# Kyaw-Thiha/animal-vision

Hardware: NVIDIA B200
Metric: Mpix/s (higher is better)
Workload: dtype f32

## Files before the change

animal_vision_b200/csrc/k3_uv.cu:

```cuda
#include <algorithm>

#include "avb_common.cuh"

namespace avb {

constexpr int UV_BINS = 2048;
constexpr int UV_NH = 3;
constexpr int UV_NR = 4;
constexpr int UV_MAX_BANDS = 160;
constexpr int UV_THREADS = 256, UV_WARPS = UV_THREADS / 32;
#ifndef UV_RH_ROWS
#define UV_RH_ROWS 64
#endif
constexpr int UV_RH = UV_RH_ROWS;
#ifndef UV_MINB
#define UV_MINB 4
#endif
#ifndef UV_HIST_WAVES
#define UV_HIST_WAVES 1
#endif
constexpr unsigned FULL = 0xffffffffu;

enum { MAP_OPPONENT = 0, MAP_FALSECOLOR = 1, MAP_MATRIX = 2, MAP_PURPLE = 3, MAP_MIXED = 4 };
enum { QS_OPP = 0, QS_UBG = 1, QS_U = 2 };

struct UvFrameStats {
    uint32_t max_bits[3];
    uint32_t pad0;
    double sum[3];
    float rcp[3];
    float pad2[6];
    float scale[3];
    float inv_w[UV_NH];
    uint32_t bin_lo[UV_NR], bin_hi[UV_NR], rank_lo[UV_NR], rank_hi[UV_NR], cand_count[UV_NR];
    float pct[UV_NR];
    uint32_t pad1;
};
static_assert(sizeof(UvFrameStats) % 8 == 0, "stats block must stay 8-byte aligned");

struct UvParams {
    FrameIO io;
    const float *lut;
    float M3[9];
    const float *bands;
    int n_bands;
    float denom_eps;
    int adapt;
    float eps;
    float t0, t1, t2;
    UvFrameStats *stats;
    uint32_t *hist;
    float *planes;
    float *cand;
    long long cap;
    const uint32_t *enc;
    int n_req;
    int req_hist[UV_NR];
    long long k_lo[UV_NR], k_hi[UV_NR];
    float gamma[UV_NR];
    int mapper;
    float map_m[9];
    float anchors[6];
    float mix_alpha;
    float *dbg_catches;
    int aligned_in, aligned_out;
    int no_plane_map;
    int strips_x, strips_y;
};

__device__ __forceinline__ float div_by(float x, float s, float r) {
    const float q = __fmul_rn(x, r);
    return fmaf(fmaf(-q, s, x), r, q);
}

__device__ __noinline__ void band_sum(const float4 *bands, int n_bands, float denom_eps, float c0, float c1, float c2,
                                      float &u, float &b, float &g) {
    float au = 0.f, ab = 0.f, ag = 0.f;
    for (int l = 0; l < n_bands; ++l) {
        const float4 lo = __ldg(bands + 2 * l), hi = __ldg(bands + 2 * l + 1);
        float spec = __fadd_rn(__fadd_rn(__fmul_rn(lo.z, c2), __fmul_rn(lo.y, c1)), __fmul_rn(lo.x, c0));
        spec = fmaxf(__fdiv_rn(spec, denom_eps), 0.f);
        const float rad = __fmul_rn(spec, lo.w);
        au = fmaf(rad, hi.x, au);
        ab = fmaf(rad, hi.y, ab);
        ag = fmaf(rad, hi.z, ag);
    }
    u = au; b = ab; g = ag;
}

template <bool BANDS>
struct Catcher {
    const float *lut_s;
    float m[9];
    const float4 *bands;
    int n_bands;
    float denom_eps;
    float sc[3], rc[3];
    bool divide;

    __device__ __forceinline__ void init_raw(const UvParams &p, const float *lut) {
        lut_s = lut;
#pragma unroll
        for (int i = 0; i < 9; ++i) m[i] = p.M3[i];
        bands = reinterpret_cast<const float4 *>(p.bands);
        n_bands = p.n_bands;
        denom_eps = p.denom_eps;
        sc[0] = sc[1] = sc[2] = 1.f;
        rc[0] = rc[1] = rc[2] = 1.f;
        divide = false;
    }
    __device__ __forceinline__ void init_adapted(const UvParams &p, const UvFrameStats &st, const float *lut) {
        init_raw(p, lut);
#pragma unroll
        for (int k = 0; k < 3; ++k) { sc[k] = st.scale[k]; rc[k] = st.rcp[k]; }
        divide = p.adapt != 0;
    }
    __device__ __forceinline__ void operator()(uint32_t b0, uint32_t b1, uint32_t b2, float &u, float &b, float &g) const {
        from_linear(lut_s[b0], lut_s[b1], lut_s[b2], u, b, g);
    }
    __device__ __forceinline__ void from_linear(float c0, float c1, float c2, float &u, float &b, float &g) const {
        if constexpr (!BANDS) {
            u = m[0] * c0 + m[1] * c1 + m[2] * c2;
            b = m[3] * c0 + m[4] * c1 + m[5] * c2;
            g = m[6] * c0 + m[7] * c1 + m[8] * c2;
            if (divide) {
                u = div_by(u, sc[0], rc[0]);
                b = div_by(b, sc[1], rc[1]);
                g = div_by(g, sc[2], rc[2]);
            }
        } else {
            float au, ab, ag;
            band_sum(bands, n_bands, denom_eps, c0, c1, c2, au, ab, ag);
            if (divide) {
                au = __fdiv_rn(au, sc[0]);
                ab = __fdiv_rn(ab, sc[1]);
                ag = __fdiv_rn(ag, sc[2]);
            }
            u = au; b = ab; g = ag;
        }
    }
};

__device__ __forceinline__ uint32_t byte_k(uint32_t w, int k) { return __byte_perm(w, 0, 0x4440 + k); }

template <class Cat>
__device__ __forceinline__ void catches4(const Cat &cat, const uint32_t (&w)[3], float (&c)[4][3]) {
    cat(byte_k(w[0], 0), byte_k(w[0], 1), byte_k(w[0], 2), c[0][0], c[0][1], c[0][2]);
    cat(byte_k(w[0], 3), byte_k(w[1], 0), byte_k(w[1], 1), c[1][0], c[1][1], c[1][2]);
    cat(byte_k(w[1], 2), byte_k(w[1], 3), byte_k(w[2], 0), c[2][0], c[2][1], c[2][2]);
    cat(byte_k(w[2], 1), byte_k(w[2], 2), byte_k(w[2], 3), c[3][0], c[3][1], c[3][2]);
}

template <int R, class Cat, class Op>
__device__ __forceinline__ void uv_walk(const UvParams &p, const Cat &cat, const uint8_t *src, int xs, int ys, int rows, Op &op) {
    constexpr int OFF = R ? 4 : 0;
    const int lane = threadIdx.x & 31;
    const int H = p.io.H, W = p.io.W;
    const int gx = xs - OFF + 4 * lane;
    const bool fast = p.aligned_in && gx >= 0 && gx + 3 < W;
    int xi[4];
#pragma unroll
    for (int j = 0; j < 4; ++j) xi[j] = 3 * reflect101(gx + j, W);
    const bool lane_ok = (R == 0) || (lane >= 1 && lane <= 30);

    auto load = [&](int i, uint32_t(&w)[3]) {
        const uint8_t *row = src + (int64_t)reflect101(ys + i, H) * p.io.in_rs;
        if (fast) {
            const uint32_t *q = reinterpret_cast<const uint32_t *>(row + 3 * gx);
            w[0] = __ldg(q); w[1] = __ldg(q + 1); w[2] = __ldg(q + 2);
        } else {
            uint32_t b[12];
#pragma unroll
            for (int j = 0; j < 4; ++j) {
                const uint8_t *q = row + xi[j];
                b[3 * j] = q[0]; b[3 * j + 1] = q[1]; b[3 * j + 2] = q[2];
            }
#pragma unroll
            for (int k = 0; k < 3; ++k) w[k] = b[4 * k] | (b[4 * k + 1] << 8) | (b[4 * k + 2] << 16) | (b[4 * k + 3] << 24);
        }
    };

    float acc[2 * R + 1][4][3];
#pragma unroll
    for (int m = 0; m < 2 * R + 1; ++m)
#pragma unroll
        for (int j = 0; j < 4; ++j)
#pragma unroll
            for (int k = 0; k < 3; ++k) acc[m][j][k] = 0.f;
    uint32_t w[3], wn[3] = {0u, 0u, 0u};
    const int n_iter = rows + 2 * R;
    const float tp[3] = {p.t0, p.t1, p.t2};
    load(-R, w);
    for (int i = 0; i < n_iter; ++i) {
        if (i + 1 < n_iter) load(i + 1 - R, wn);
        float c[4][3];
        catches4(cat, w, c);
        float v[4][3];
        if constexpr (R == 0) {
#pragma unroll
            for (int j = 0; j < 4; ++j)
#pragma unroll
                for (int k = 0; k < 3; ++k) v[j][k] = c[j][k];
        } else {
#pragma unroll
            for (int k = 0; k < 3; ++k) {
                float e[8];
                e[1] = __shfl_up_sync(FULL, c[3][k], 1);
                e[6] = __shfl_down_sync(FULL, c[0][k], 1);
                if (R == 2) {
                    e[0] = __shfl_up_sync(FULL, c[2][k], 1);
                    e[7] = __shfl_down_sync(FULL, c[1][k], 1);
                } else {
                    e[0] = e[7] = 0.f;
                }
#pragma unroll
                for (int j = 0; j < 4; ++j) e[2 + j] = c[j][k];
#pragma unroll
                for (int j = 0; j < 4; ++j) {
                    float h = fmaf(tp[1], e[1 + j] + e[3 + j], tp[0] * e[2 + j]);
                    if (R == 2) h = fmaf(tp[2], e[j] + e[4 + j], h);
                    v[j][k] = fmaf(tp[R], h, acc[0][j][k]);
#pragma unroll
                    for (int m = 0; m < 2 * R - 1; ++m) {
                        const int d = (R - 1 - m) < 0 ? -(R - 1 - m) : (R - 1 - m);
                        acc[m][j][k] = fmaf(tp[d], h, acc[m + 1][j][k]);
                    }
                    acc[2 * R - 1][j][k] = tp[R] * h;
                }
            }
        }
        if (i >= 2 * R) op(ys + i - 2 * R, gx, v, lane_ok);
#pragma unroll
        for (int k = 0; k < 3; ++k) w[k] = wn[k];
    }
}

template <int R>
__device__ __forceinline__ void strip_of(const UvParams &p, int task, int &xs, int &ys, int &rows) {
    constexpr int SW = R ? 120 : 128;
    const int sy = task / p.strips_x, sx = task - sy * p.strips_x;
    xs = sx * SW;
    ys = sy * UV_RH;
    rows = min(UV_RH, p.io.H - ys);
}

__device__ __forceinline__ float sqrt_sfu(float x) {
#ifdef UV_SQRT_RN
    return __fsqrt_rn(x);
#else
    float r;
    asm("sqrt.approx.ftz.f32 %0, %1;" : "=f"(r) : "f"(x));
    return r;
#endif
}

__device__ __forceinline__ float atan2_fast(float y, float x) {
    const float ax = fabsf(x), ay = fabsf(y);
    const float mx = fmaxf(ax, ay), mn = fminf(ax, ay);
    const float a = mx > 0.f ? __fdividef(mn, mx) : 0.f;
    const float s = a * a;
    float r = 0.0028662257f;
    r = fmaf(r, s, -0.0161657367f);
    r = fmaf(r, s, 0.0429096138f);
    r = fmaf(r, s, -0.0752896400f);
    r = fmaf(r, s, 0.1065626393f);
    r = fmaf(r, s, -0.1420889944f);
    r = fmaf(r, s, 0.1999355085f);
// ... 8 lines not shown
__device__ __forceinline__ float opp_hue(const float (&c)[3]) {
    const float O1 = c[2] - c[1], O2 = c[1] - c[0];
    const float PI_F = 3.14159274101257324f;
    const float ang = PRECISE ? atan2f(O2, O1) : atan2_fast(O2, O1);
    return div_by(__fadd_rn(ang, PI_F), 6.28318548202514648f, 0.159154936671257019f);
}

template <int QS, bool PRECISE = false>
__device__ __forceinline__ void quantities(const float (&c)[3], float (&q)[UV_NH]) {
    if (QS == QS_OPP) {
        const float O1 = c[2] - c[1], O2 = c[1] - c[0];
        const float r2 = __fadd_rn(__fmul_rn(O1, O1), __fmul_rn(O2, O2));
        q[0] = PRECISE ? __fsqrt_rn(r2) : sqrt_sfu(r2);
        q[1] = div_by(__fadd_rn(__fadd_rn(c[0], c[1]), c[2]), 3.0f, 0.333333343267440796f);
        q[2] = 0.f;
    } else {
        q[0] = c[0]; q[1] = c[1]; q[2] = c[2];
    }
}
template <int QS>
struct QCount { static constexpr int value = QS == QS_OPP ? 2 : (QS == QS_UBG ? 3 : 1); };

__device__ __forceinline__ int bin_of(float v, float inv_w) {
    return min(UV_BINS - 1, max(0, __float2int_rd(v * inv_w)));
}

template <bool BANDS>
__global__ void __launch_bounds__(256) uv_stats_kernel(const __grid_constant__ UvParams p) {
    __shared__ float lut_s[256];
    for (int i = threadIdx.x; i < 256; i += blockDim.x) lut_s[i] = __ldg(p.lut + i);
    __syncthreads();
    const int frame = blockIdx.y;
    const uint8_t *src = p.io.in + (int64_t)frame * p.io.in_fs;
    Catcher<BANDS> cat;
    cat.init_raw(p, lut_s);
    float mx[3] = {0.f, 0.f, 0.f};
    double sm[3] = {0.0, 0.0, 0.0};
    const int W = p.io.W, H = p.io.H;
    const int groups = (W + 3) >> 2;
    for (int y = blockIdx.x; y < H; y += gridDim.x) {
        const uint8_t *row = src + (int64_t)y * p.io.in_rs;
        float rs[3] = {0.f, 0.f, 0.f};
        int gi = threadIdx.x;
        if (p.aligned_in) {
            for (; gi + 3 * (int)blockDim.x < groups - 1; gi += 4 * blockDim.x) {
                uint32_t w[4][3];
#pragma unroll
                for (int u = 0; u < 4; ++u) {
                    const uint32_t *q = reinterpret_cast<const uint32_t *>(row + 12 * (gi + u * (int)blockDim.x));
                    w[u][0] = __ldg(q); w[u][1] = __ldg(q + 1); w[u][2] = __ldg(q + 2);
                }
#pragma unroll
                for (int u = 0; u < 4; ++u) {
                    float c[4][3];
                    catches4(cat, w[u], c);
#pragma unroll
                    for (int j = 0; j < 4; ++j) {
#pragma unroll
                        for (int k = 0; k < 3; ++k) {
                            mx[k] = fmaxf(mx[k], c[j][k]);
                            rs[k] += c[j][k];
                        }
                        if (p.dbg_catches) {
                            float *d = p.dbg_catches + (((int64_t)frame * H + y) * W + 4 * (gi + u * (int)blockDim.x) + j) * 3;
                            d[0] = c[j][0]; d[1] = c[j][1]; d[2] = c[j][2];
                        }
                    }
                }
// ... 21 lines not shown
                    d[0] = c[j][0]; d[1] = c[j][1]; d[2] = c[j][2];
                }
            }
        }
#pragma unroll
        for (int k = 0; k < 3; ++k) sm[k] += (double)rs[k];
    }
    __shared__ float red_m[8][3];
    __shared__ double red_s[8][3];
    const int lane = threadIdx.x & 31, wid = threadIdx.x >> 5;
#pragma unroll
    for (int k = 0; k < 3; ++k) {
        float m = mx[k];
        double s = sm[k];
#pragma unroll
        for (int o = 16; o > 0; o >>= 1) {
            m = fmaxf(m, __shfl_xor_sync(FULL, m, o));
            s += __shfl_xor_sync(FULL, s, o);
        }
        if (lane == 0) { red_m[wid][k] = m; red_s[wid][k] = s; }
    }
    __syncthreads();
    if (threadIdx.x < 3) {
        const int k = threadIdx.x;
        float m = 0.f;
        double s = 0.0;
        for (int w = 0; w < (int)(blockDim.x >> 5); ++w) { m = fmaxf(m, red_m[w][k]); s += red_s[w][k]; }
        UvFrameStats &st = p.stats[frame];
        atomicMax(&st.max_bits[k], __float_as_uint(fmaxf(m, 0.f)));
        atomicAdd(&st.sum[k], s);
    }
}

template <int QS>
__global__ void uv_prep_kernel(const __grid_constant__ UvParams p) {
    const int frame = blockIdx.x * blockDim.x + threadIdx.x;
    if (frame >= p.io.n) return;
    UvFrameStats &st = p.stats[frame];
    const double npx = (double)p.io.H * (double)p.io.W;
    float ub[3];
#pragma unroll
    for (int k = 0; k < 3; ++k) {
        const float mx = __uint_as_float(st.max_bits[k]);
        float s = 1.0f;
        if (p.adapt == 1) s = fmaxf(mx, p.eps);
        else if (p.adapt == 2) s = fmaxf((float)(st.sum[k] / npx), p.eps);
        st.scale[k] = s;
        st.rcp[k] = __frcp_rn(s);
        ub[k] = mx / s * 1.001f + 1e-30f;
    }
    float hb[UV_NH];
    if (QS == QS_OPP) {
        const float a = fmaxf(ub[2], ub[1]), b = fmaxf(ub[1], ub[0]);
        hb[0] = sqrtf(a * a + b * b) * 1.001f;
        hb[1] = (ub[0] + ub[1] + ub[2]) * (1.001f / 3.0f);
        hb[2] = 1.f;
    } else {
        hb[0] = ub[0]; hb[1] = ub[1]; hb[2] = ub[2];
    }
#pragma unroll
    for (int h = 0; h < UV_NH; ++h) st.inv_w[h] = (float)UV_BINS / fmaxf(hb[h], 1e-30f);
}

__host__ __device__ __forceinline__ bool map_from_planes(const UvParams &p) {
    return p.n_req > 0 && (p.io.W & 3) == 0 && p.aligned_out != 0 && !p.no_plane_map;
}

template <int QS>
struct HistOp {
    uint32_t *hs;
    float *planes;
    long long npx;
    float inv_w[UV_NH];
    int W;
    bool vec;
    bool hue_plane;
    __device__ __forceinline__ void operator()(int y, int gx, const float (&v)[4][3], bool ok) {
        if (!ok || gx >= W) return;
        constexpr int NPL = QS == QS_OPP ? 3 : QCount<QS>::value;
        float q[4][UV_NH];
        const bool full = gx + 3 < W;
#pragma unroll
        for (int j = 0; j < 4; ++j) {
            quantities<QS>(v[j], q[j]);
            if (QS == QS_OPP && hue_plane) q[j][2] = opp_hue<false>(v[j]);
        }
        if (full) {
#pragma unroll
            for (int j = 0; j < 4; ++j)
#pragma unroll
                for (int h = 0; h < QCount<QS>::value; ++h) atomicAdd(&hs[h * UV_BINS + bin_of(q[j][h], inv_w[h])], 1u);
        } else {
#pragma unroll
            for (int j = 0; j < 4; ++j)
                if (gx + j < W) {
#pragma unroll
                    for (int h = 0; h < QCount<QS>::value; ++h) atomicAdd(&hs[h * UV_BINS + bin_of(q[j][h], inv_w[h])], 1u);
                }
        }
        const long long o = (long long)y * W + gx;
#pragma unroll
        for (int h = 0; h < NPL; ++h) {
            if (h >= QCount<QS>::value && !hue_plane) break;
            float *d = planes + h * npx + o;
            if (vec) {
                *reinterpret_cast<float4 *>(d) = make_float4(q[0][h], q[1][h], q[2][h], q[3][h]);
            } else {
#pragma unroll
                for (int j = 0; j < 4; ++j)
                    if (gx + j < W) d[j] = q[j][h];
            }
        }
    }
};

template <int QS, int R, bool BANDS>
__global__ void __launch_bounds__(UV_THREADS, UV_MINB) uv_hist_kernel(const __grid_constant__ UvParams p) {
    __shared__ float lut_s[256];
    __shared__ uint32_t hs[QCount<QS>::value * UV_BINS];
    const int tid = threadIdx.x, frame = blockIdx.y;
    for (int i = tid; i < 256; i += UV_THREADS) lut_s[i] = __ldg(p.lut + i);
    for (int i = tid; i < QCount<QS>::value * UV_BINS; i += UV_THREADS) hs[i] = 0u;
    __syncthreads();
    const UvFrameStats &st = p.stats[frame];
    Catcher<BANDS> cat;
    cat.init_adapted(p, st, lut_s);
    HistOp<QS> op;
    op.hs = hs;
    op.npx = (long long)p.io.H * p.io.W;
    op.planes = p.planes + (long long)frame * UV_NH * op.npx;
    op.vec = (p.io.W & 3) == 0;
    op.hue_plane = map_from_planes(p);
#pragma unroll
    for (int h = 0; h < UV_NH; ++h) op.inv_w[h] = st.inv_w[h];
    op.W = p.io.W;
    const uint8_t *src = p.io.in + (int64_t)frame * p.io.in_fs;
    const int tasks = p.strips_x * p.strips_y;
    for (int task = blockIdx.x * UV_WARPS + (tid >> 5); task < tasks; task += gridDim.x * UV_WARPS) {
        int xs, ys, rows;
        strip_of<R>(p, task, xs, ys, rows);
        uv_walk<R>(p, cat, src, xs, ys, rows, op);
    }
    __syncthreads();
    uint32_t *gh = p.hist + (int64_t)frame * UV_NH * UV_BINS;
    for (int i = tid; i < QCount<QS>::value * UV_BINS; i += UV_THREADS) {
        const uint32_t c = hs[i];
        if (c) atomicAdd(gh + i, c);
    }
}

__global__ void __launch_bounds__(256) uv_scan_kernel(const __grid_constant__ UvParams p) {
    const int frame = blockIdx.x, tid = threadIdx.x;
    UvFrameStats &st = p.stats[frame];
    __shared__ uint32_t part[256];
    __shared__ uint32_t res[4];
    constexpr int PER = UV_BINS / 256;
    for (int r = 0; r < p.n_req; ++r) {
        const uint32_t *h = p.hist + ((int64_t)frame * UV_NH + p.req_hist[r]) * UV_BINS;
        const uint32_t k_lo = (uint32_t)p.k_lo[r], k_hi = (uint32_t)p.k_hi[r];
        uint32_t loc[PER], s = 0;
#pragma unroll
        for (int j = 0; j < PER; ++j) { loc[j] = h[tid * PER + j]; s += loc[j]; }
        part[tid] = s;
        __syncthreads();
        if (tid == 0) {
            uint32_t run = 0;
            for (int i = 0; i < 256; ++i) { const uint32_t v = part[i]; part[i] = run; run += v; }
        }
        __syncthreads();
        uint32_t run = part[tid];
#pragma unroll
        for (int j = 0; j < PER; ++j) {
            if (k_lo >= run && k_lo < run + loc[j]) { res[0] = tid * PER + j; res[1] = run; }
            if (k_hi >= run && k_hi < run + loc[j]) res[2] = tid * PER + j;
// ... 208 lines not shown
    EncTable enc;
    uint8_t *dst;
    int64_t out_rs;
    int W;
    bool aligned;
    __device__ __forceinline__ void operator()(int y, int gx, const float (&v)[4][3], bool ok) {
        if (!ok || gx >= W) return;
        uint32_t by[12];
#pragma unroll
        for (int j = 0; j < 4; ++j) {
            float rgb[3];
            map_pixel<MAPPER>(v[j], k, rgb);
#pragma unroll
            for (int i = 0; i < 3; ++i) by[3 * j + i] = encode_u8(enc, rgb[i]);
        }
        uint8_t *o = dst + (int64_t)y * out_rs + 3 * gx;
        if (aligned && gx + 3 < W) {
            uint32_t *o32 = reinterpret_cast<uint32_t *>(o);
#pragma unroll
            for (int q = 0; q < 3; ++q) o32[q] = by[4 * q] | (by[4 * q + 1] << 8) | (by[4 * q + 2] << 16) | (by[4 * q + 3] << 24);
        } else {
            const int nb = 3 * min(4, W - gx);
#pragma unroll
            for (int q = 0; q < 12; ++q)
                if (q < nb) o[q] = (uint8_t)by[q];
        }
    }
};

template <int MAPPER, int R, bool BANDS>
__global__ void __launch_bounds__(UV_THREADS, UV_MINB) uv_map_kernel(const __grid_constant__ UvParams p) {
    __shared__ float lut_s[256];
    __shared__ uint32_t enc_s[AVB_ENC_TABLE_MAX];
    const int tid = threadIdx.x, frame = blockIdx.y;
    for (int i = tid; i < 256; i += UV_THREADS) lut_s[i] = __ldg(p.lut + i);
    copy_to_smem(enc_s, p.enc, min((int)AVB_ENC_TABLE_MAX, ENC_HEADER + (int)__ldg(p.enc + 2)));
    __syncthreads();
    const UvFrameStats &st = p.stats[frame];
    Catcher<BANDS> cat;
    cat.init_adapted(p, st, lut_s);
    MapOp<MAPPER> op;
    op.enc = enc_view(enc_s);
    op.dst = p.io.out + (int64_t)frame * p.io.out_fs;
    op.out_rs = p.io.out_rs;
    op.W = p.io.W;
    op.aligned = p.aligned_out != 0;
    MapConsts &k = op.k;
    k.pr = st.pct[0] + p.eps;
    k.pL = st.pct[1] + p.eps;
    k.rpr = __frcp_rn(k.pr);
    k.rpL = __frcp_rn(k.pL);
#pragma unroll
    for (int i = 0; i < 3; ++i) { k.d95[i] = fmaxf(st.pct[i], p.eps); k.r95[i] = __frcp_rn(k.d95[i]); }
    k.d98 = fmaxf(MAPPER == MAP_PURPLE ? st.pct[0] : st.pct[3], p.eps);
    k.r98 = __frcp_rn(k.d98);
#pragma unroll
    for (int i = 0; i < 3; ++i) {
        k.c0[i] = p.anchors[i];
        k.c1[i] = p.anchors[3 + i];
        k.pd[i] = __fsub_rn(k.c0[i], 0.5f);
        k.m[3 * i] = p.map_m[3 * i]; k.m[3 * i + 1] = p.map_m[3 * i + 1]; k.m[3 * i + 2] = p.map_m[3 * i + 2];
    }
    k.alpha = p.mix_alpha;
    const uint8_t *src = p.io.in + (int64_t)frame * p.io.in_fs;
    const int tasks = p.strips_x * p.strips_y;
    for (int task = blockIdx.x * UV_WARPS + (tid >> 5); task < tasks; task += gridDim.x * UV_WARPS) {
        int xs, ys, rows;
        strip_of<R>(p, task, xs, ys, rows);
        uv_walk<R>(p, cat, src, xs, ys, rows, op);
    }
}


__device__ __forceinline__ void fill_map_consts(const UvParams &p, const UvFrameStats &st, int mapper, MapConsts &k) {
    k.pr = st.pct[0] + p.eps;
    k.pL = st.pct[1] + p.eps;
    k.rpr = __frcp_rn(k.pr);
    k.rpL = __frcp_rn(k.pL);
#pragma unroll
    for (int i = 0; i < 3; ++i) { k.d95[i] = fmaxf(st.pct[i], p.eps); k.r95[i] = __frcp_rn(k.d95[i]); }
    k.d98 = fmaxf(mapper == MAP_PURPLE ? st.pct[0] : st.pct[3], p.eps);
    k.r98 = __frcp_rn(k.d98);
#pragma unroll
    for (int i = 0; i < 3; ++i) {
        k.c0[i] = p.anchors[i];
        k.c1[i] = p.anchors[3 + i];
        k.pd[i] = __fsub_rn(k.c0[i], 0.5f);
        k.m[3 * i] = p.map_m[3 * i]; k.m[3 * i + 1] = p.map_m[3 * i + 1]; k.m[3 * i + 2] = p.map_m[3 * i + 2];
    }
    k.alpha = p.mix_alpha;
}

constexpr int MP_THREADS = 256, MP_GROUPS = 4;
#ifndef MP_MINB
#define MP_MINB 4
#endif
template <int MAPPER>
__global__ void __launch_bounds__(MP_THREADS, MP_MINB) uv_map_planes_kernel(const __grid_constant__ UvParams p) {
    constexpr int NPL = MAPPER == MAP_PURPLE ? 1 : 3;
    __shared__ uint32_t enc_s[AVB_ENC_TABLE_MAX];
    const int tid = threadIdx.x, frame = blockIdx.y;
    copy_to_smem(enc_s, p.enc, min((int)AVB_ENC_TABLE_MAX, ENC_HEADER + (int)__ldg(p.enc + 2)));
// ... 36 lines not shown
        const float h4[4] = {qh[u].x, qh[u].y, qh[u].z, qh[u].w};
        uint32_t by[12];
#pragma unroll
        for (int j = 0; j < 4; ++j) {
            float rgb[3];
            if (MAPPER == MAP_OPPONENT) {
                opp_color(r4[j], L4[j], h4[j], k, rgb);
            } else {
                const float c[3] = {r4[j], L4[j], h4[j]};
                map_pixel<MAPPER>(c, k, rgb);
            }
#pragma unroll
            for (int i = 0; i < 3; ++i) by[3 * j + i] = encode_u8(enc, rgb[i]);
        }
        uint32_t *o32 = reinterpret_cast<uint32_t *>(dst + (int64_t)y * p.io.out_rs + 12u * x4);
#pragma unroll
        for (int q = 0; q < 3; ++q) o32[q] = by[4 * q] | (by[4 * q + 1] << 8) | (by[4 * q + 2] << 16) | (by[4 * q + 3] << 24);
    }
}

__device__ __forceinline__ float srgb_decode_torch(float t) {
    return t <= 0.04045f ? __fdiv_rn(t, 12.92f) : powf(__fdiv_rn(t + 0.055f, 1.055f), 2.4f);
}
__device__ __forceinline__ float srgb_encode_uv(float l) {
    return l <= 0.0031308f ? __fmul_rn(l, 12.92f) : __fsub_rn(__fmul_rn(1.055f, powf(fmaxf(l, 0.f), 0.41666666f)), 0.055f);
}

struct CatchF32P {
    const float *in; float *out; long long npx;
    UvParams uv;
};
template <bool BANDS>
__global__ void __launch_bounds__(256) uv_catches_f32_kernel(const __grid_constant__ CatchF32P p) {
    Catcher<BANDS> cat;
    cat.init_raw(p.uv, nullptr);
    for (long long i = (long long)blockIdx.x * 256 + threadIdx.x; i < p.npx; i += (long long)gridDim.x * 256) {
        const float c0 = srgb_decode_torch(p.in[3 * i]), c1 = srgb_decode_torch(p.in[3 * i + 1]), c2 = srgb_decode_torch(p.in[3 * i + 2]);
        float u, b, g;
        cat.from_linear(c0, c1, c2, u, b, g);
        p.out[3 * i] = u; p.out[3 * i + 1] = b; p.out[3 * i + 2] = g;
    }
}

struct PlaneP {
    const float *ubg;
    void *out;
    int out_f32, quantize;
    UvParams uv;
};

__global__ void __launch_bounds__(256) uv_planemax_kernel(const __grid_constant__ PlaneP p) {
    const int frame = blockIdx.y;
    const long long npx = (long long)p.uv.io.H * p.uv.io.W;
    const float *f = p.ubg + (long long)frame * npx * 3;
    float m[3] = {0.f, 0.f, 0.f};
    for (long long i = (long long)blockIdx.x * 256 + threadIdx.x; i < npx; i += (long long)gridDim.x * 256) {
#pragma unroll
        for (int k = 0; k < 3; ++k) m[k] = fmaxf(m[k], f[3 * i + k]);
    }
#pragma unroll
    for (int k = 0; k < 3; ++k) {
#pragma unroll
        for (int o = 16; o > 0; o >>= 1) m[k] = fmaxf(m[k], __shfl_xor_sync(FULL, m[k], o));
        if ((threadIdx.x & 31) == 0) atomicMax(&p.uv.stats[frame].max_bits[k], __float_as_uint(m[k]));
    }
}

template <int QS>
__global__ void __launch_bounds__(256) uv_hist_f32_kernel(const __grid_constant__ PlaneP p) {
    __shared__ uint32_t hs[QCount<QS>::value * UV_BINS];
    const int tid = threadIdx.x, frame = blockIdx.y;
    for (int i = tid; i < QCount<QS>::value * UV_BINS; i += 256) hs[i] = 0u;
// ... 80 lines not shown
        }
        {
            AVB_TIMED("k3_uv_select", st);
            uv_select_kernel<<<dim3(p.n_req, p.io.n), SEL_THREADS, 0, st>>>(p);
        }
    }
    {
        AVB_TIMED("k3_uv_map_f32", st);
        uv_map_f32_kernel<MAPPER><<<dim3(bx, p.io.n), 256, 0, st>>>(pp);
    }
    AVB_CUDA_OK(cudaGetLastError());
    return AVB_OK;
}

static int qset_of(int mapper) {
    switch (mapper) {
        case MAP_OPPONENT: return QS_OPP;
        case MAP_PURPLE: return QS_U;
        default: return QS_UBG;
    }
}

static dim3 walk_grid(const UvParams &p, int per_sm) {
    const int tasks = p.strips_x * p.strips_y;
    int bx = (tasks + UV_WARPS - 1) / UV_WARPS;
    const int cap = sm_count() * per_sm / p.io.n;
    if (bx > cap) bx = cap < 1 ? 1 : cap;
    return dim3(bx, p.io.n);
}

template <int QS, int R, bool BANDS>
static int launch_percentiles(const UvParams &p, cudaStream_t st) {
    {
        AVB_TIMED("k3_uv_hist", st);
        uv_hist_kernel<QS, R, BANDS><<<walk_grid(p, 4 * UV_HIST_WAVES), UV_THREADS, 0, st>>>(p);
    }
    {
        AVB_TIMED("k3_uv_scan", st);
        uv_scan_kernel<<<p.io.n, 256, 0, st>>>(p);
    }
    {
        AVB_TIMED("k3_uv_compact", st);
        const long long npx = (long long)p.io.H * p.io.W;
        uv_compact_kernel<<<dim3((unsigned)((npx + CP_PER_BLOCK - 1) / CP_PER_BLOCK), p.n_req, p.io.n), 256, 0, st>>>(p);
    }
    {
        AVB_TIMED("k3_uv_select", st);
        uv_select_kernel<<<dim3(p.n_req, p.io.n), SEL_THREADS, 0, st>>>(p);
    }
    AVB_CUDA_OK(cudaGetLastError());
    return AVB_OK;
}

template <int MAPPER, int R, bool BANDS>
static int launch_mapper(const UvParams &p, cudaStream_t st) {
    constexpr int QS = MAPPER == MAP_OPPONENT ? QS_OPP : (MAPPER == MAP_PURPLE ? QS_U : QS_UBG);
    {
        AVB_TIMED("k3_uv_prep", st);
        uv_prep_kernel<QS><<<(p.io.n + 63) / 64, 64, 0, st>>>(p);
    }
    if (p.n_req > 0)
        if (int e = launch_percentiles<QS, R, BANDS>(p, st)) return e;
    if (MAPPER != MAP_MATRIX && map_from_planes(p)) {
        AVB_TIMED("k3_uv_map", st);
        const long long groups = ((long long)p.io.H * p.io.W) >> 2, per_cta = (long long)MP_THREADS * MP_GROUPS;
        uv_map_planes_kernel<MAPPER><<<dim3((unsigned)((groups + per_cta - 1) / per_cta), p.io.n), MP_THREADS, 0, st>>>(p);
    } else {
        AVB_TIMED("k3_uv_map", st);
        const int tasks = p.strips_x * p.strips_y;
        uv_map_kernel<MAPPER, R, BANDS><<<dim3((tasks + UV_WARPS - 1) / UV_WARPS, p.io.n), UV_THREADS, 0, st>>>(p);
    }
    AVB_CUDA_OK(cudaGetLastError());
    return AVB_OK;
}

template <int R, bool BANDS>
static int dispatch_mapper(const UvParams &p, cudaStream_t st) {
    switch (p.mapper) {
        case MAP_OPPONENT: return launch_mapper<MAP_OPPONENT, R, BANDS>(p, st);
        case MAP_FALSECOLOR: return launch_mapper<MAP_FALSECOLOR, R, BANDS>(p, st);
        case MAP_MATRIX: return launch_mapper<MAP_MATRIX, R, BANDS>(p, st);
        case MAP_PURPLE: return launch_mapper<MAP_PURPLE, R, BANDS>(p, st);
        default: return launch_mapper<MAP_MIXED, R, BANDS>(p, st);
    }
}

static int n_requests(int mapper) {
    switch (mapper) {
        case MAP_OPPONENT: return 2;
        case MAP_FALSECOLOR: return 3;
        case MAP_MATRIX: return 0;
        case MAP_PURPLE: return 1;
        default: return 4;
    }
}

static size_t align_up(size_t v, size_t a) { return (v + a - 1) / a * a; }

}

using namespace avb;

extern "C" int64_t avb_uv_workspace_bytes(int n, int H, int W, int map_mode) {
    if (n <= 0 || H <= 0 || W <= 0 || map_mode < 0 || map_mode > MAP_MIXED) return 0;
    const size_t stats = align_up((size_t)n * sizeof(UvFrameStats), 256);
    const size_t hist = (size_t)n * UV_NH * UV_BINS * sizeof(uint32_t);
    const size_t planes = n_requests(map_mode) ? (size_t)n * UV_NH * (size_t)H * W * sizeof(float) : 0;
    const size_t cand = (size_t)n * n_requests(map_mode) * (size_t)H * W * sizeof(float);
    return (int64_t)(stats + hist + planes + cand);
}

extern "C" int avb_uv_map_u8(const uint8_t *in, uint8_t *out, int n, int H, int W,
                             int64_t in_frame_stride, int64_t in_row_stride,
                             int64_t out_frame_stride, int64_t out_row_stride,
                             const float *dec_dev, const uint32_t *enc_dev,
                             const float *m3_host, const float *bands_dev, int n_bands, float denom_eps,
                             int adapt_mode, const float *blur_taps_host, int blur_ksize,
                             int map_mode, const float *map_params_host, float mix_alpha,
                             void *workspace_dev, float *dbg_catches_dev, avb_stream_t stream) {
    UvParams p{};
    p.io = FrameIO{in, out, in_frame_stride, in_row_stride, out_frame_stride, out_row_stride, n, H, W};
    AVB_REQUIRE(in && out, "null frame pointer");
    AVB_REQUIRE(n > 0 && H > 0 && W > 0, "bad frame geometry");
    AVB_REQUIRE(n <= 65535, "batch too large for one launch");
    AVB_REQUIRE(in_row_stride >= 3LL * W && out_row_stride >= 3LL * W, "row stride smaller than 3*W");
    AVB_REQUIRE(dec_dev && enc_dev && m3_host && workspace_dev, "null table / workspace pointer");
    AVB_REQUIRE((reinterpret_cast<uintptr_t>(workspace_dev) & 15) == 0, "workspace_dev must be 16-byte aligned (float4 plane accesses)");
    AVB_REQUIRE(n_bands >= 0 && n_bands <= UV_MAX_BANDS && (n_bands == 0 || bands_dev), "bad band table");
    AVB_REQUIRE(adapt_mode >= 0 && adapt_mode <= 2, "adapt_mode must be 0 (none), 1 (white patch) or 2 (gray world)");
    AVB_REQUIRE(blur_ksize == 0 || ((blur_ksize == 3 || blur_ksize == 5) && blur_taps_host), "blur ksize must be 0, 3 or 5");
// ... 23 lines not shown
    p.aligned_in = ((reinterpret_cast<uintptr_t>(in) | (uintptr_t)in_frame_stride | (uintptr_t)in_row_stride) & 3) == 0;
    p.aligned_out = ((reinterpret_cast<uintptr_t>(out) | (uintptr_t)out_frame_stride | (uintptr_t)out_row_stride) & 3) == 0;
    {
        static const bool off = [] { const char *e = std::getenv("AVB_UV_NO_PLANE_MAP"); return e && e[0] == '1'; }();
        p.no_plane_map = off ? 1 : 0;
    }
    const int SW = R ? 120 : 128;
    p.strips_x = (W + SW - 1) / SW;
    p.strips_y = (H + UV_RH - 1) / UV_RH;

    const long long npx = (long long)H * W;
    uint8_t *ws = static_cast<uint8_t *>(workspace_dev);
    const size_t stats_bytes = align_up((size_t)n * sizeof(UvFrameStats), 256);
    const size_t hist_bytes = (size_t)n * UV_NH * UV_BINS * sizeof(uint32_t);
    p.stats = reinterpret_cast<UvFrameStats *>(ws);
    p.hist = reinterpret_cast<uint32_t *>(ws + stats_bytes);
    const size_t planes_bytes = n_requests(map_mode) ? (size_t)n * UV_NH * (size_t)npx * sizeof(float) : 0;
    p.planes = reinterpret_cast<float *>(ws + stats_bytes + hist_bytes);
    p.cand = reinterpret_cast<float *>(ws + stats_bytes + hist_bytes + planes_bytes);
    p.cap = npx;

    p.n_req = n_requests(map_mode);
    const int qs = qset_of(map_mode);
    const double pcts[5][UV_NR] = {{95, 95, 0, 0}, {95, 95, 95, 0}, {0, 0, 0, 0}, {98, 0, 0, 0}, {95, 95, 95, 98}};
    const int hists[5][UV_NR] = {{0, 1, 0, 0}, {0, 1, 2, 0}, {0, 0, 0, 0}, {0, 0, 0, 0}, {0, 1, 2, 0}};
    (void)qs;
    for (int r = 0; r < p.n_req; ++r) {
        const PctIndex pi = numpy_percentile_index(pcts[map_mode][r], npx);
        p.req_hist[r] = hists[map_mode][r];
        p.k_lo[r] = pi.k_lo; p.k_hi[r] = pi.k_hi; p.gamma[r] = pi.gamma;
    }

    AVB_CUDA_OK(cudaMemsetAsync(ws, 0, stats_bytes + hist_bytes, st));
    {
        int bx = (sm_count() * 16 + n - 1) / n;
        if (bx > H) bx = H;
        dim3 grid((unsigned)bx, n);
        AVB_TIMED("k3_uv_stats", st);
        if (n_bands) uv_stats_kernel<true><<<grid, 256, 0, st>>>(p);
        else uv_stats_kernel<false><<<grid, 256, 0, st>>>(p);
        AVB_CUDA_OK(cudaGetLastError());
    }
    if (n_bands) {
        switch (R) {
            case 0: return dispatch_mapper<0, true>(p, st);
            case 1: return dispatch_mapper<1, true>(p, st);
            default: return dispatch_mapper<2, true>(p, st);
        }
    }
    switch (R) {
        case 0: return dispatch_mapper<0, false>(p, st);
        case 1: return dispatch_mapper<1, false>(p, st);
        default: return dispatch_mapper<2, false>(p, st);
    }
}

extern "C" int avb_uv_catches_f32(const float *img01_dev, float *catches_dev, int64_t npx, const float *m3_host,
                                  const float *bands_dev, int n_bands, float denom_eps, avb_stream_t stream) {
    AVB_REQUIRE(img01_dev && catches_dev && m3_host, "null pointer");
    AVB_REQUIRE(npx > 0, "bad geometry");
    AVB_REQUIRE(n_bands >= 0 && n_bands <= UV_MAX_BANDS && (n_bands == 0 || bands_dev), "bad band table");
    cudaStream_t st = static_cast<cudaStream_t>(stream);
    CatchF32P p{};
    p.in = img01_dev; p.out = catches_dev; p.npx = npx;
    for (int i = 0; i < 9; ++i) p.uv.M3[i] = m3_host[i];
    p.uv.bands = bands_dev; p.uv.n_bands = n_bands; p.uv.denom_eps = denom_eps;
    const unsigned bx = (unsigned)std::max<long long>(1, std::min<long long>((npx + 255) / 256, (long long)sm_count() * 16));
// ... 59 lines not shown
```

Before: 117,300.

## Add dedicated max-reduction stats kernel, replicated LUT, dynamic hist scheduling, fast-path templating

When the input is 16-byte aligned and W is a multiple of 16, the stats pass is replaced by a lightweight max-only kernel. It uses 128-bit loads and a 32-way replicated shared LUT to avoid bank conflicts. The histogram kernel gains atomic work-stealing via a next_task counter in the stats block, and uses the replicated LUT when it has two or fewer queues. uv_walk now selects the aligned fast path per strip as a template parameter, and Catcher is slimmed to reference params instead of copying them, applying adaptation after gathering. Risks include larger shared memory lowering occupancy, extra atomics, and skipping the sums the old stats kernel computed when the fast path is taken.

```diff
diff --git a/animal_vision_b200/csrc/k3_uv.cu b/animal_vision_b200/csrc/k3_uv.cu
--- a/animal_vision_b200/csrc/k3_uv.cu
+++ b/animal_vision_b200/csrc/k3_uv.cu
@@ -26,7 +26,7 @@
 
 struct UvFrameStats {
     uint32_t max_bits[3];
-    uint32_t pad0;
+    uint32_t next_task;
     double sum[3];
     float rcp[3];
     float pad2[6];
@@ -37,6 +37,7 @@
     uint32_t pad1;
 };
 static_assert(sizeof(UvFrameStats) % 8 == 0, "stats block must stay 8-byte aligned");
+static_assert(sizeof(UvFrameStats) == 200, "tests/test_gpu_uv_stats.py reads max_bits from 200-byte records");
 
 struct UvParams {
     FrameIO io;
@@ -88,56 +89,37 @@
     u = au; b = ab; g = ag;
 }
 
-template <bool BANDS>
+constexpr int LUT_REP = 32;
+__device__ __forceinline__ void fill_lut_rep(float *dst, const float *lut) {
+    for (int i = threadIdx.x; i < 256 * LUT_REP; i += blockDim.x) dst[i] = __ldg(lut + i / LUT_REP);
+}
+
+template <bool BANDS, bool REP = false>
 struct Catcher {
+    static constexpr int LS = REP ? LUT_REP : 1;
+    const UvParams &p;
     const float *lut_s;
-    float m[9];
-    const float4 *bands;
-    int n_bands;
-    float denom_eps;
-    float sc[3], rc[3];
+    const float2 *sr;
     bool divide;
 
-    __device__ __forceinline__ void init_raw(const UvParams &p, const float *lut) {
-        lut_s = lut;
-#pragma unroll
-        for (int i = 0; i < 9; ++i) m[i] = p.M3[i];
-        bands = reinterpret_cast<const float4 *>(p.bands);
-        n_bands = p.n_bands;
-        denom_eps = p.denom_eps;
-        sc[0] = sc[1] = sc[2] = 1.f;
-        rc[0] = rc[1] = rc[2] = 1.f;
-        divide = false;
-    }
-    __device__ __forceinline__ void init_adapted(const UvParams &p, const UvFrameStats &st, const float *lut) {
-        init_raw(p, lut);
-#pragma unroll
-        for (int k = 0; k < 3; ++k) { sc[k] = st.scale[k]; rc[k] = st.rcp[k]; }
-        divide = p.adapt != 0;
-    }
+    __device__ __forceinline__ Catcher(const UvParams &params, const float *lut, const float2 *scale_rcp = nullptr)
+        : p(params), lut_s(lut), sr(scale_rcp), divide(scale_rcp != nullptr && params.adapt != 0) {}
     __device__ __forceinline__ void operator()(uint32_t b0, uint32_t b1, uint32_t b2, float &u, float &b, float &g) const {
-        from_linear(lut_s[b0], lut_s[b1], lut_s[b2], u, b, g);
-    }
-    __device__ __forceinline__ void from_linear(float c0, float c1, float c2, float &u, float &b, float &g) const {
+        raw(lut_s[b0 * LS], lut_s[b1 * LS], lut_s[b2 * LS], u, b, g);
+    }
+    __device__ __forceinline__ void raw(float c0, float c1, float c2, float &u, float &b, float &g) const {
         if constexpr (!BANDS) {
+            const float *m = p.M3;
             u = m[0] * c0 + m[1] * c1 + m[2] * c2;
             b = m[3] * c0 + m[4] * c1 + m[5] * c2;
             g = m[6] * c0 + m[7] * c1 + m[8] * c2;
-            if (divide) {
-                u = div_by(u, sc[0], rc[0]);
-                b = div_by(b, sc[1], rc[1]);
-                g = div_by(g, sc[2], rc[2]);
-            }
         } else {
-            float au, ab, ag;
-            band_sum(bands, n_bands, denom_eps, c0, c1, c2, au, ab, ag);
-            if (divide) {
-                au = __fdiv_rn(au, sc[0]);
-                ab = __fdiv_rn(ab, sc[1]);
-                ag = __fdiv_rn(ag, sc[2]);
-            }
-            u = au; b = ab; g = ag;
-        }
+            band_sum(reinterpret_cast<const float4 *>(p.bands), p.n_bands, p.denom_eps, c0, c1, c2, u, b, g);
+        }
+    }
+    __device__ __forceinline__ void adapt(float (&c)[3], const float2 (&s)[3]) const {
+#pragma unroll
+        for (int k = 0; k < 3; ++k) c[k] = BANDS ? __fdiv_rn(c[k], s[k].x) : div_by(c[k], s[k].x, s[k].y);
     }
 };
 
@@ -149,30 +131,31 @@
     cat(byte_k(w[0], 3), byte_k(w[1], 0), byte_k(w[1], 1), c[1][0], c[1][1], c[1][2]);
     cat(byte_k(w[1], 2), byte_k(w[1], 3), byte_k(w[2], 0), c[2][0], c[2][1], c[2][2]);
     cat(byte_k(w[2], 1), byte_k(w[2], 2), byte_k(w[2], 3), c[3][0], c[3][1], c[3][2]);
-}
-
-template <int R, class Cat, class Op>
+    if (cat.divide) {
+        const float2 s[3] = {cat.sr[0], cat.sr[1], cat.sr[2]};
+#pragma unroll
+        for (int j = 0; j < 4; ++j) cat.adapt(c[j], s);
+    }
+}
+
+template <int R, bool FAST, class Cat, class Op>
 __device__ __forceinline__ void uv_walk(const UvParams &p, const Cat &cat, const uint8_t *src, int xs, int ys, int rows, Op &op) {
     constexpr int OFF = R ? 4 : 0;
     const int lane = threadIdx.x & 31;
     const int H = p.io.H, W = p.io.W;
     const int gx = xs - OFF + 4 * lane;
-    const bool fast = p.aligned_in && gx >= 0 && gx + 3 < W;
-    int xi[4];
-#pragma unroll
-    for (int j = 0; j < 4; ++j) xi[j] = 3 * reflect101(gx + j, W);
-    const bool lane_ok = (R == 0) || (lane >= 1 && lane <= 30);
-
-    auto load = [&](int i, uint32_t(&w)[3]) {
-        const uint8_t *row = src + (int64_t)reflect101(ys + i, H) * p.io.in_rs;
-        if (fast) {
+    const bool lane_ok = ((R == 0) || (lane >= 1 && lane <= 30)) && gx < W;
+
+    auto load = [&](int y, uint32_t(&w)[3]) {
+        const uint8_t *row = src + (int64_t)reflect101(y, H) * p.io.in_rs;
+        if (FAST) {
             const uint32_t *q = reinterpret_cast<const uint32_t *>(row + 3 * gx);
             w[0] = __ldg(q); w[1] = __ldg(q + 1); w[2] = __ldg(q + 2);
         } else {
             uint32_t b[12];
 #pragma unroll
             for (int j = 0; j < 4; ++j) {
-                const uint8_t *q = row + xi[j];
+                const uint8_t *q = row + 3 * reflect101(gx + j, W);
                 b[3 * j] = q[0]; b[3 * j + 1] = q[1]; b[3 * j + 2] = q[2];
             }
 #pragma unroll
@@ -188,11 +171,11 @@
 #pragma unroll
             for (int k = 0; k < 3; ++k) acc[m][j][k] = 0.f;
     uint32_t w[3], wn[3] = {0u, 0u, 0u};
-    const int n_iter = rows + 2 * R;
-    const float tp[3] = {p.t0, p.t1, p.t2};
-    load(-R, w);
-    for (int i = 0; i < n_iter; ++i) {
-        if (i + 1 < n_iter) load(i + 1 - R, wn);
+    auto tp = [&](int d) { return d == 0 ? p.t0 : (d == 1 ? p.t1 : p.t2); };
+    load(ys - R, w);
+    const int y_end = ys + rows + R;
+    for (int y = ys - R; y < y_end; ++y) {
+        if (y + 1 < y_end) load(y + 1, wn);
         float c[4][3];
         catches4(cat, w, c);
         float v[4][3];
@@ -217,22 +200,28 @@
                 for (int j = 0; j < 4; ++j) e[2 + j] = c[j][k];
 #pragma unroll
                 for (int j = 0; j < 4; ++j) {
-                    float h = fmaf(tp[1], e[1 + j] + e[3 + j], tp[0] * e[2 + j]);
-                    if (R == 2) h = fmaf(tp[2], e[j] + e[4 + j], h);
-                    v[j][k] = fmaf(tp[R], h, acc[0][j][k]);
+                    float h = fmaf(tp(1), e[1 + j] + e[3 + j], tp(0) * e[2 + j]);
+                    if (R == 2) h = fmaf(tp(2), e[j] + e[4 + j], h);
+                    v[j][k] = fmaf(tp(R), h, acc[0][j][k]);
 #pragma unroll
                     for (int m = 0; m < 2 * R - 1; ++m) {
                         const int d = (R - 1 - m) < 0 ? -(R - 1 - m) : (R - 1 - m);
-                        acc[m][j][k] = fmaf(tp[d], h, acc[m + 1][j][k]);
+                        acc[m][j][k] = fmaf(tp(d), h, acc[m + 1][j][k]);
                     }
-                    acc[2 * R - 1][j][k] = tp[R] * h;
+                    acc[2 * R - 1][j][k] = tp(R) * h;
                 }
             }
         }
-        if (i >= 2 * R) op(ys + i - 2 * R, gx, v, lane_ok);
+        if (y >= ys + R) op(y - R, gx, v, lane_ok);
 #pragma unroll
         for (int k = 0; k < 3; ++k) w[k] = wn[k];
     }
+}
+
+template <int R>
+__device__ __forceinline__ bool strip_fast(const UvParams &p, int xs) {
+    constexpr int OFF = R ? 4 : 0;
+    return p.aligned_in && xs - OFF >= 0 && xs - OFF + 4 * 31 + 3 < p.io.W;
 }
 
 template <int R>
@@ -307,8 +296,7 @@
     __syncthreads();
     const int frame = blockIdx.y;
     const uint8_t *src = p.io.in + (int64_t)frame * p.io.in_fs;
-    Catcher<BANDS> cat;
-    cat.init_raw(p, lut_s);
+    Catcher<BANDS> cat(p, lut_s);
     float mx[3] = {0.f, 0.f, 0.f};
     double sm[3] = {0.0, 0.0, 0.0};
     const int W = p.io.W, H = p.io.H;
@@ -396,6 +384,62 @@
     }
 }
 
+constexpr int MX_THREADS = 256, MX_CHUNKS = 4;
+template <bool BANDS>
+__global__ void __launch_bounds__(MX_THREADS) uv_max_kernel(const __grid_constant__ UvParams p) {
+    __shared__ float lut_s[256 * LUT_REP];
+    __shared__ float red[MX_THREADS / 32][3];
+    fill_lut_rep(lut_s, p.lut);
+    __syncthreads();
+    const Catcher<BANDS, true> cat(p, lut_s + (threadIdx.x & 31));
+    const uint8_t *src = p.io.in + (int64_t)blockIdx.y * p.io.in_fs;
+    const uint32_t per_row = (uint32_t)p.io.W >> 4, chunks = per_row * (uint32_t)p.io.H;
+    const uint32_t stride = gridDim.x * MX_THREADS;
+    float mx[3] = {0.f, 0.f, 0.f};
+    for (uint32_t c0 = blockIdx.x * MX_THREADS + threadIdx.x; c0 < chunks; c0 += MX_CHUNKS * stride) {
+        uint4 q[MX_CHUNKS][3];
+#pragma unroll
+        for (int u = 0; u < MX_CHUNKS; ++u) {
+            const uint32_t c = c0 + u * stride;
+            if (c < chunks) {
+                const uint32_t y = c / per_row, x = c - y * per_row;
+                const uint4 *s = reinterpret_cast<const uint4 *>(src + (int64_t)y * p.io.in_rs + 48 * x);
+                q[u][0] = __ldg(s); q[u][1] = __ldg(s + 1); q[u][2] = __ldg(s + 2);
+            }
+        }
+#pragma unroll
+        for (int u = 0; u < MX_CHUNKS; ++u) {
+            if (c0 + u * stride >= chunks) break;
+            const uint32_t w[12] = {q[u][0].x, q[u][0].y, q[u][0].z, q[u][0].w, q[u][1].x, q[u][1].y,
+                                    q[u][1].z, q[u][1].w, q[u][2].x, q[u][2].y, q[u][2].z, q[u][2].w};
+#pragma unroll
+            for (int g = 0; g < 4; ++g) {
+                float c[4][3];
+                catches4(cat, {w[3 * g], w[3 * g + 1], w[3 * g + 2]}, c);
+#pragma unroll
+                for (int j = 0; j < 4; ++j)
+#pragma unroll
+                    for (int k = 0; k < 3; ++k) mx[k] = fmaxf(mx[k], c[j][k]);
+            }
+        }
+    }
+    const int lane = threadIdx.x & 31, wid = threadIdx.x >> 5;
+#pragma unroll
+    for (int k = 0; k < 3; ++k) {
+        float m = mx[k];
+#pragma unroll
+        for (int o = 16; o > 0; o >>= 1) m = fmaxf(m, __shfl_xor_sync(FULL, m, o));
+        if (lane == 0) red[wid][k] = m;
+    }
+    __syncthreads();
+    if (threadIdx.x < 3) {
+        const int k = threadIdx.x;
+        float m = 0.f;
+        for (int w = 0; w < MX_THREADS / 32; ++w) m = fmaxf(m, red[w][k]);
+        atomicMax(&p.stats[blockIdx.y].max_bits[k], __float_as_uint(fmaxf(m, 0.f)));
+    }
+}
+
 template <int QS>
 __global__ void uv_prep_kernel(const __grid_constant__ UvParams p) {
     const int frame = blockIdx.x * blockDim.x + threadIdx.x;
@@ -432,15 +476,16 @@
 
 template <int QS>
 struct HistOp {
+    const UvParams &p;
     uint32_t *hs;
-    float *planes;
-    long long npx;
-    float inv_w[UV_NH];
-    int W;
-    bool vec;
-    bool hue_plane;
+    const float *inv_w;
     __device__ __forceinline__ void operator()(int y, int gx, const float (&v)[4][3], bool ok) {
+        const int W = p.io.W;
         if (!ok || gx >= W) return;
+        const long long npx = (long long)p.io.H * W;
+        const bool vec = (W & 3) == 0;
+        const bool hue_plane = map_from_planes(p);
+        float *planes = p.planes + (long long)blockIdx.y * UV_NH * npx;
         constexpr int NPL = QS == QS_OPP ? 3 : QCount<QS>::value;
         float q[4][UV_NH];
         const bool full = gx + 3 < W;
@@ -478,32 +523,42 @@
     }
 };
 
+template <int QS>
+struct HistLutRep { static constexpr bool value = QCount<QS>::value <= 2; };
+template <int QS>
+constexpr int hist_smem_bytes() { return HistLutRep<QS>::value ? 256 * LUT_REP * (int)sizeof(float) : 0; }
+
 template <int QS, int R, bool BANDS>
 __global__ void __launch_bounds__(UV_THREADS, UV_MINB) uv_hist_kernel(const __grid_constant__ UvParams p) {
-    __shared__ float lut_s[256];
+    constexpr bool REP = HistLutRep<QS>::value;
+    extern __shared__ float lut_dyn[];
+    __shared__ float lut_one[REP ? 1 : 256];
+    float *lut_s = REP ? lut_dyn : lut_one;
     __shared__ uint32_t hs[QCount<QS>::value * UV_BINS];
+    __shared__ float inv_w_s[UV_NH];
+    __shared__ float2 sr_s[3];
     const int tid = threadIdx.x, frame = blockIdx.y;
-    for (int i = tid; i < 256; i += UV_THREADS) lut_s[i] = __ldg(p.lut + i);
+    const UvFrameStats &st = p.stats[frame];
+    if (REP) fill_lut_rep(lut_s, p.lut);
+    else
+        for (int i = tid; i < 256; i += UV_THREADS) lut_s[i] = __ldg(p.lut + i);
     for (int i = tid; i < QCount<QS>::value * UV_BINS; i += UV_THREADS) hs[i] = 0u;
-    __syncthreads();
-    const UvFrameStats &st = p.stats[frame];
-    Catcher<BANDS> cat;
-    cat.init_adapted(p, st, lut_s);
-    HistOp<QS> op;
-    op.hs = hs;
-    op.npx = (long long)p.io.H * p.io.W;
-    op.planes = p.planes + (long long)frame * UV_NH * op.npx;
-    op.vec = (p.io.W & 3) == 0;
-    op.hue_plane = map_from_planes(p);
-#pragma unroll
-    for (int h = 0; h < UV_NH; ++h) op.inv_w[h] = st.inv_w[h];
-    op.W = p.io.W;
+    if (tid < UV_NH) inv_w_s[tid] = st.inv_w[tid];
+    if (tid < 3) sr_s[tid] = make_float2(st.scale[tid], st.rcp[tid]);
+    __syncthreads();
+    Catcher<BANDS, REP> cat(p, REP ? lut_s + (tid & 31) : lut_s, sr_s);
+    HistOp<QS> op{p, hs, inv_w_s};
     const uint8_t *src = p.io.in + (int64_t)frame * p.io.in_fs;
     const int tasks = p.strips_x * p.strips_y;
-    for (int task = blockIdx.x * UV_WARPS + (tid >> 5); task < tasks; task += gridDim.x * UV_WARPS) {
+    int task = blockIdx.x * UV_WARPS + (tid >> 5);
+    while (task < tasks) {
         int xs, ys, rows;
         strip_of<R>(p, task, xs, ys, rows);
-        uv_walk<R>(p, cat, src, xs, ys, rows, op);
+        if (strip_fast<R>(p, xs)) uv_walk<R, true>(p, cat, src, xs, ys, rows, op);
+        else uv_walk<R, false>(p, cat, src, xs, ys, rows, op);
+        int next = 0;
+        if ((tid & 31) == 0) next = (int)atomicAdd(&p.stats[frame].next_task, 1u);
+        task = gridDim.x * UV_WARPS + __shfl_sync(FULL, next, 0);
     }
     __syncthreads();
     uint32_t *gh = p.hist + (int64_t)frame * UV_NH * UV_BINS;
@@ -778,13 +833,14 @@
 __global__ void __launch_bounds__(UV_THREADS, UV_MINB) uv_map_kernel(const __grid_constant__ UvParams p) {
     __shared__ float lut_s[256];
     __shared__ uint32_t enc_s[AVB_ENC_TABLE_MAX];
+    __shared__ float2 sr_s[3];
     const int tid = threadIdx.x, frame = blockIdx.y;
+    const UvFrameStats &st = p.stats[frame];
     for (int i = tid; i < 256; i += UV_THREADS) lut_s[i] = __ldg(p.lut + i);
     copy_to_smem(enc_s, p.enc, min((int)AVB_ENC_TABLE_MAX, ENC_HEADER + (int)__ldg(p.enc + 2)));
-    __syncthreads();
-    const UvFrameStats &st = p.stats[frame];
-    Catcher<BANDS> cat;
-    cat.init_adapted(p, st, lut_s);
+    if (tid < 3) sr_s[tid] = make_float2(st.scale[tid], st.rcp[tid]);
+    __syncthreads();
+    Catcher<BANDS> cat(p, lut_s, sr_s);
     MapOp<MAPPER> op;
     op.enc = enc_view(enc_s);
     op.dst = p.io.out + (int64_t)frame * p.io.out_fs;
@@ -813,7 +869,8 @@
     for (int task = blockIdx.x * UV_WARPS + (tid >> 5); task < tasks; task += gridDim.x * UV_WARPS) {
         int xs, ys, rows;
         strip_of<R>(p, task, xs, ys, rows);
-        uv_walk<R>(p, cat, src, xs, ys, rows, op);
+        if (strip_fast<R>(p, xs)) uv_walk<R, true>(p, cat, src, xs, ys, rows, op);
+        else uv_walk<R, false>(p, cat, src, xs, ys, rows, op);
     }
 }
 
@@ -916,12 +973,11 @@
 };
 template <bool BANDS>
 __global__ void __launch_bounds__(256) uv_catches_f32_kernel(const __grid_constant__ CatchF32P p) {
-    Catcher<BANDS> cat;
-    cat.init_raw(p.uv, nullptr);
+    Catcher<BANDS> cat(p.uv, nullptr);
     for (long long i = (long long)blockIdx.x * 256 + threadIdx.x; i < p.npx; i += (long long)gridDim.x * 256) {
         const float c0 = srgb_decode_torch(p.in[3 * i]), c1 = srgb_decode_torch(p.in[3 * i + 1]), c2 = srgb_decode_torch(p.in[3 * i + 2]);
         float u, b, g;
-        cat.from_linear(c0, c1, c2, u, b, g);
+        cat.raw(c0, c1, c2, u, b, g);
         p.out[3 * i] = u; p.out[3 * i + 1] = b; p.out[3 * i + 2] = g;
     }
 }
@@ -1068,8 +1124,10 @@
 template <int QS, int R, bool BANDS>
 static int launch_percentiles(const UvParams &p, cudaStream_t st) {
     {
+        static SmemOptIn opt;
+        AVB_CUDA_OK(opt.ensure(uv_hist_kernel<QS, R, BANDS>, hist_smem_bytes<QS>()));
         AVB_TIMED("k3_uv_hist", st);
-        uv_hist_kernel<QS, R, BANDS><<<walk_grid(p, 4 * UV_HIST_WAVES), UV_THREADS, 0, st>>>(p);
+        uv_hist_kernel<QS, R, BANDS><<<walk_grid(p, 4 * UV_HIST_WAVES), UV_THREADS, hist_smem_bytes<QS>(), st>>>(p);
     }
     {
         AVB_TIMED("k3_uv_scan", st);
@@ -1132,6 +1190,23 @@
 }
 
 static size_t align_up(size_t v, size_t a) { return (v + a - 1) / a * a; }
+
+template <bool BANDS>
+static int launch_max(const UvParams &p, cudaStream_t st) {
+    static std::atomic<int> per_sm{0};
+    int r = per_sm.load();
+    if (r == 0) {
+        AVB_CUDA_OK(cudaOccupancyMaxActiveBlocksPerMultiprocessor(&r, uv_max_kernel<BANDS>, MX_THREADS, 0));
+        r = std::max(r, 1);
+        per_sm.store(r);
+    }
+    const long long chunks = (long long)p.io.H * (p.io.W >> 4);
+    const long long bx = std::max(1LL, std::min<long long>((long long)sm_count() * r / p.io.n, (chunks + MX_THREADS - 1) / MX_THREADS));
+    AVB_TIMED("k3_uv_stats", st);
+    uv_max_kernel<BANDS><<<dim3((unsigned)bx, p.io.n), MX_THREADS, 0, st>>>(p);
+    AVB_CUDA_OK(cudaGetLastError());
+    return AVB_OK;
+}
 
 }
 
@@ -1221,7 +1296,10 @@
     }
 
     AVB_CUDA_OK(cudaMemsetAsync(ws, 0, stats_bytes + hist_bytes, st));
-    {
+    const bool rows16 = ((reinterpret_cast<uintptr_t>(in) | (uintptr_t)in_frame_stride | (uintptr_t)in_row_stride) & 15) == 0;
+    if (adapt_mode != 2 && !dbg_catches_dev && rows16 && W % 16 == 0) {
+        if (int e = n_bands ? launch_max<true>(p, st) : launch_max<false>(p, st)) return e;
+    } else {
         int bx = (sm_count() * 16 + n - 1) / n;
         if (bx > H) bx = H;
         dim3 grid((unsigned)bx, n);
```

Result: faster. 120,400, median of 6 (+2.7%).
